# oharari/Convex-Combination-of-Gaussian-Processes

Measured on AMD Instinct MI355X. Metric: GP log-lik evals/sec (n x n fp64, batched over hyperpar grid), higher is better.
Workload: dtype f64; 1 GPU; cfg4: synthetic maximin-LHS 5-D design n=4096, K=3 anisotropic components, 512-point hyperparameter grid sharded over the GPUs; n=4096, d=5, K=3, evals_total=512, evals_per_gpu=512, parallelism=grid sharded over 1 GPU(s), one all-gather

## Files before the change

convex-combination-of-gaussian-processes_amd/csrc/blocked.hip:

```cpp
#include <cstdlib>
#include <vector>

#include "ccgp_internal.h"
#include "sched_logic.h"

namespace ccgp {

typedef double d4 __attribute__((ext_vector_type(4)));

namespace {

__device__ __forceinline__ int tid_now() {
  int t = threadIdx.x;
  asm volatile("" : "+v"(t));
  return t;
}

__device__ __forceinline__ constexpr int swz_src(int l, int parity) { return (((l >> 3) ^ parity) << 4) + ((l & 7) << 1); }

struct GemmArgs {
  double* A;
  size_t a_stride;
  int npad;
  double* invd;
  size_t invd_stride;
  int j, nt, nb;
  int ld;
  int ne;
  int extra_lower;
  int mode;
  double* E;
  size_t e_stride;
  int lde;
  int rows_only;
  int fuse_diag;
  int tail_strips;
  int wide;
  int n_s1;
  int tail_s;
  double* logdet_part;
  int* status;
  int n;
  double ptol;
};

template <int S, bool THIN>
struct TileGeom {
  static constexpr int CW = kTile / S;
  static constexpr int NX = THIN ? (S == 1 ? 2 : 1) : (S == 1 ? 4 : 2);
  static constexpr int NY = THIN ? 1 : (S == 4 ? 2 : 4);
  static constexpr int BK = 16;
  __device__ static int row0(int wave) { return THIN ? 0 : (S == 4 ? wave * 32 : (wave >> 1) * 64); }
  __device__ static int col0(int wave) {
    return THIN ? wave * NX * 16 : (S == 4 ? 0 : (wave & 1) * (S == 1 ? 64 : 32));
  }
};

template <int S, bool THIN, bool TRI>
__device__ __forceinline__ int col_block(int wave, int x) {
  if constexpr (TRI && !THIN) return (wave & 1) + 2 * x;
  else return (TileGeom<S, THIN>::col0(wave) >> 4) + x;
}

template <bool IL>
struct AccMap {
  int row0, col0, l15, l4;
  __device__ __forceinline__ AccMap() {
    const int lane = tid_now() & 63, wave = tid_now() >> 6;
    row0 = TileGeom<1, false>::row0(wave); col0 = TileGeom<1, false>::col0(wave); l15 = lane & 15; l4 = lane >> 4;
  }
  __device__ __forceinline__ int row(int y) const { return IL ? row0 + 4 * l15 + y : row0 + 16 * y + l15; }
  __device__ __forceinline__ int col(int x, int r) const { return IL ? col0 + 16 * r + 4 * l4 + x : col0 + 16 * x + l4 + 4 * r; }
  static constexpr __device__ __forceinline__ int dcol(int x, int r) { return IL ? 16 * r + x : 16 * x + 4 * r; }
  __device__ __forceinline__ double* lane_base(double* C, int ld) const {
    return IL ? C + row0 + 4 * l15 + (size_t)(col0 + 4 * l4) * ld : C + row0 + l15 + (size_t)(col0 + l4) * ld;
  }
};

template <int S, bool THIN, bool TRI = false>
__device__ __forceinline__ void gemm_accumulate(double* smem, const double* P, int ldP, const double* Q,
                                                int ldQ, int Kdim,
                                                d4 (&acc)[TileGeom<S, THIN>::NX][TileGeom<S, THIN>::NY]) {
  static_assert(!TRI || S == 1, "the triangular skip is only wired for full-width tiles");
  constexpr int CW = TileGeom<S, THIN>::CW;
  constexpr int NX = TileGeom<S, THIN>::NX;
  constexpr int NY = TileGeom<S, THIN>::NY;
  constexpr int BKs = TileGeom<S, THIN>::BK;
  constexpr int STAGE = BKs * kTile + BKs * CW;
  constexpr int CPI = kTile / CW;
  constexpr int QI = BKs / CPI / 4;
  const int tid = tid_now(), lane = tid & 63, wave = tid >> 6;
  const int row0 = TileGeom<S, THIN>::row0(wave);
  const int col0 = TileGeom<S, THIN>::col0(wave);
  const bool active = !THIN || col0 < CW;
  const int l15 = lane & 15, l4 = lane >> 4;

#pragma unroll
  for (int x = 0; x < NX; ++x)
#pragma unroll
    for (int y = 0; y < NY; ++y) acc[x][y] = d4{0.0, 0.0, 0.0, 0.0};

  const double* pP = P + swz_src(lane, wave & 1) + (size_t)wave * ldP;
  const size_t stepP = (size_t)4 * ldP;
  constexpr int LPC = 64 / CPI;
  const int qcol_in = lane / LPC, ql = lane % LPC;
  const int qpar = CPI == 1 ? (wave & 1) : (qcol_in & 1);
  const double* pQ = Q + swz_src(ql, qpar) + (size_t)(CPI * wave + qcol_in) * ldQ;
  const size_t stepQ = (size_t)(4 * CPI) * ldQ;

  auto issue = [&](int stage) {
    double* Ps_ = smem + stage * STAGE + wave * kTile;
    double* Qs_ = smem + stage * STAGE + BKs * kTile + wave * kTile;
#pragma unroll
    for (int q = 0; q < BKs / 4; ++q)
      __builtin_amdgcn_global_load_lds((const __attribute__((address_space(1))) void*)(pP + q * stepP),
                                       (__attribute__((address_space(3))) void*)(Ps_ + 4 * q * kTile), 16, 0, 0);
#pragma unroll
    for (int q = 0; q < QI; ++q)
      __builtin_amdgcn_global_load_lds((const __attribute__((address_space(1))) void*)(pQ + q * stepQ),
                                       (__attribute__((address_space(3))) void*)(Qs_ + 4 * q * kTile), 16, 0, 0);
    pP += (BKs / 4) * stepP;
    pQ += QI * stepQ;
  };

  static_assert(BKs == 16, "the pipeline below is written for four k-steps per stage");
  double pfA[NY], qfA[NX], pfB[NY], qfB[NX];
  const int sw = l4 & 1;
#define CCGP_LOADF(PF, QF, STG, KK)                                                              \
  do {                                                                                          \
    const double* Ps_ = smem + (STG) * STAGE;                                                   \
    const double* Qs_ = Ps_ + BKs * kTile;                                                      \
    _Pragma("unroll") for (int y = 0; y < NY; ++y)                                              \
        PF[y] = Ps_[((KK) * 4 + l4) * kTile + ((((row0 >> 4) + y) ^ sw) << 4) + l15];           \
    _Pragma("unroll") for (int x = 0; x < NX; ++x)                                              \
        QF[x] = Qs_[((KK) * 4 + l4) * CW + ((col_block<S, THIN, TRI>(wave, x) ^ sw) << 4) + l15]; \
    __builtin_amdgcn_sched_barrier(0);                                                          \
  } while (0)
#define CCGP_MFMAS(PF, QF, KT, X0, X1)                                                           \
  do {                                                                                          \
    if (active) {                                                                               \
      _Pragma("unroll") for (int x = (X0); x < (X1); ++x) {                                     \
        if (TRI && col_block<S, THIN, TRI>(wave, x) * 16 + 15 < (KT) * BKs) continue;           \
        _Pragma("unroll") for (int y = 0; y < NY; ++y)                                          \
            acc[x][y] = __builtin_amdgcn_mfma_f64_16x16x4f64(QF[x], PF[y], acc[x][y], 0, 0, 0); \
      }                                                                                         \
    }                                                                                           \
    __builtin_amdgcn_sched_barrier(0);                                                          \
  } while (0)
  constexpr int XH = NX > 1 ? 1 : NX;

  const int nk = Kdim / BKs;
  issue(0);
  __syncthreads();
  if (nk > 1) issue(1);
  CCGP_LOADF(pfA, qfA, 0, 0);
  for (int kt = 0; kt < nk; ++kt) {
    const int stg = kt & 1;
    CCGP_MFMAS(pfA, qfA, kt, 0, XH);
    CCGP_LOADF(pfB, qfB, stg, 1);
    CCGP_MFMAS(pfA, qfA, kt, XH, NX);
    CCGP_MFMAS(pfB, qfB, kt, 0, XH);
    CCGP_LOADF(pfA, qfA, stg, 2);
    CCGP_MFMAS(pfB, qfB, kt, XH, NX);
    CCGP_MFMAS(pfA, qfA, kt, 0, XH);
    CCGP_LOADF(pfB, qfB, stg, 3);
    CCGP_MFMAS(pfA, qfA, kt, XH, NX);
    if (kt + 1 < nk) {
      __syncthreads();
      if (kt + 2 < nk) issue(stg);
    }
    CCGP_MFMAS(pfB, qfB, kt, 0, XH);
// ... 201 lines not shown
#pragma unroll
        for (int t = 0; t < 2; ++t)
#pragma unroll
          for (int r = 0; r < 4; ++r) Co[t * 16 + (size_t)(gr.cb * 16 + 4 * r) * ld] = o[gr.cb][t][r];
      }
      __builtin_amdgcn_sched_barrier(0);
    }
  };
  struct Half0 { SolveGroup v[26]; };
  struct Half1 { SolveGroup v[10]; };
  constexpr Half0 h0{{{0, 0}, {1, 0}, {1, 1}, {2, 0}, {2, 1}, {2, 2}, {3, 0}, {3, 1}, {3, 2}, {3, 3},
                      {4, 0}, {4, 1}, {4, 2}, {4, 3}, {5, 0}, {5, 1}, {5, 2}, {5, 3},
                      {6, 0}, {6, 1}, {6, 2}, {6, 3}, {7, 0}, {7, 1}, {7, 2}, {7, 3}}};
  constexpr Half1 h1{{{4, 4}, {5, 4}, {5, 5}, {6, 4}, {6, 5}, {6, 6}, {7, 4}, {7, 5}, {7, 6}, {7, 7}}};

  __syncthreads();
  if ((wave & 1) == 0) dump();
  __syncthreads();
  run(h0, 0);
  __syncthreads();
  if ((wave & 1) == 1) dump();
  __syncthreads();
  run(h1, 1);
}

template <int S>
__device__ __forceinline__ void strip_accumulate_ring(double* smem, const double* P, int ldP, const double* Q, int ldQ,
                                                      int Kdim,
                                                      d4 (&acc)[TileGeom<S, false>::NX][TileGeom<S, false>::NY]) {
  static_assert(S == 2 || S == 4, "the ring exists for half- and quarter-width strips");
  constexpr int BKd = 8, NST = 4;
  constexpr int CW = TileGeom<S, false>::CW, NX = TileGeom<S, false>::NX, NY = TileGeom<S, false>::NY;
  static_assert(NX == 2, "the stage loop below splits a k-step's MFMAs at x = 1");
  constexpr int STAGE = BKd * kTile + BKd * CW;
  const int tid = tid_now(), lane = tid & 63, wave = tid >> 6;
  const int row0 = TileGeom<S, false>::row0(wave), col0 = TileGeom<S, false>::col0(wave);
  const int l15 = lane & 15, l4 = lane >> 4;
#pragma unroll
  for (int x = 0; x < NX; ++x)
#pragma unroll
    for (int y = 0; y < NY; ++y) acc[x][y] = d4{0.0, 0.0, 0.0, 0.0};

  const double* pP = P + swz_src(lane, wave & 1) + (size_t)wave * ldP;
  constexpr int LPR = CW / 2;
  const int ql = lane & (LPR - 1), qrow = lane / LPR;
  const int qw = S == 2 ? wave : (wave & 1);
  const double* pQ = Q + swz_src(ql, qrow & 1) + (size_t)(S * qw + qrow) * ldQ;
  auto issue = [&](int slot) {
    double* Ps_ = smem + slot * STAGE + wave * kTile;
    double* Qs_ = smem + slot * STAGE + BKd * kTile + qw * S * CW;
    __builtin_amdgcn_global_load_lds((const __attribute__((address_space(1))) void*)pP,
                                     (__attribute__((address_space(3))) void*)Ps_, 16, 0, 0);
    __builtin_amdgcn_global_load_lds((const __attribute__((address_space(1))) void*)(pP + (size_t)4 * ldP),
                                     (__attribute__((address_space(3))) void*)(Ps_ + 4 * kTile), 16, 0, 0);
    __builtin_amdgcn_global_load_lds((const __attribute__((address_space(1))) void*)pQ,
                                     (__attribute__((address_space(3))) void*)Qs_, 16, 0, 0);
    pP += (size_t)BKd * ldP;
    pQ += (size_t)BKd * ldQ;
  };
  auto wait_and_meet = [&](int later_stages) {
    if (later_stages >= 3) __builtin_amdgcn_s_waitcnt(0x0079);
    else if (later_stages == 2) __builtin_amdgcn_s_waitcnt(0x0076);
    else if (later_stages == 1) __builtin_amdgcn_s_waitcnt(0x0073);
    else __builtin_amdgcn_s_waitcnt(0x0070);
    __builtin_amdgcn_s_barrier();
  };

  const int sw = l4 & 1;
  const int offP = l4 * kTile + l15, offQ = BKd * kTile + l4 * CW + l15;
  int rbo[NY], cbo[NX];
#pragma unroll
  for (int t = 0; t < NY; ++t) rbo[t] = (((row0 >> 4) + t) ^ sw) << 4;
#pragma unroll
  for (int t = 0; t < NX; ++t) cbo[t] = (((col0 >> 4) + t) ^ sw) << 4;
  double pfA[NY], qfA[NX], pfB[NY], qfB[NX];
#define CCGP_RLOADF(PF, QF, SLOT, KK)                                                            \
  do {                                                                                          \
    const double* St_ = smem + (SLOT) * STAGE;                                                  \
    _Pragma("unroll") for (int y = 0; y < NY; ++y) PF[y] = St_[(KK) * 4 * kTile + offP + rbo[y]]; \
    _Pragma("unroll") for (int x = 0; x < NX; ++x) QF[x] = St_[(KK) * 4 * CW + offQ + cbo[x]];  \
    __builtin_amdgcn_sched_barrier(0);                                                          \
  } while (0)
#define CCGP_RMFMAS(PF, QF, X0, X1)                                                              \
  do {                                                                                          \
    _Pragma("unroll") for (int x = (X0); x < (X1); ++x)                                         \
      _Pragma("unroll") for (int y = 0; y < NY; ++y)                                            \
          acc[x][y] = __builtin_amdgcn_mfma_f64_16x16x4f64(QF[x], PF[y], acc[x][y], 0, 0, 0);   \
    __builtin_amdgcn_sched_barrier(0);                                                          \
  } while (0)

  const int nk = Kdim / BKd;
  const int pre = nk < NST ? nk : NST;
  for (int t = 0; t < pre; ++t) issue(t);
  __builtin_amdgcn_sched_barrier(0);
  wait_and_meet(pre - 1);
  CCGP_RLOADF(pfA, qfA, 0, 0);
  for (int kt = 0; kt < nk; ++kt) {
    const int slot = kt & (NST - 1);
    CCGP_RLOADF(pfB, qfB, slot, 1);
    CCGP_RMFMAS(pfA, qfA, 0, 2);
    if (kt + 1 < nk) {
      const int last_issued = kt + NST - 1 < nk - 1 ? kt + NST - 1 : nk - 1;
      wait_and_meet(last_issued - (kt + 1));
      if (kt + NST < nk) issue(slot);
      __builtin_amdgcn_sched_barrier(0);
    }
    CCGP_RMFMAS(pfB, qfB, 0, 1);
    if (kt + 1 < nk) CCGP_RLOADF(pfA, qfA, (kt + 1) & (NST - 1), 0);
    CCGP_RMFMAS(pfB, qfB, 1, 2);
  }
#undef CCGP_RLOADF
#undef CCGP_RMFMAS
}

template <int S, bool THIN, bool TRI = false, bool RING = false>
__device__ __forceinline__ void gemm_tile(double* smem, const double* P, int ldP, const double* Q,
                                          int ldQ, int Kdim, double* C, int ld, int mode) {
  constexpr int NX = TileGeom<S, THIN>::NX;
  constexpr int NY = TileGeom<S, THIN>::NY;
  d4 acc[NX][NY];
  if constexpr (RING) {
    static_assert((S == 2 || S == 4) && !THIN && !TRI, "the four-stage ring exists for half- and quarter-width update strips");
    strip_accumulate_ring<S>(smem, P, ldP, Q, ldQ, Kdim, acc);
  } else {
    gemm_accumulate<S, THIN, TRI>(smem, P, ldP, Q, ldQ, Kdim, acc);
  }
  const int lane = tid_now() & 63, wave = tid_now() >> 6;
  const int row0 = TileGeom<S, THIN>::row0(wave), col0 = TileGeom<S, THIN>::col0(wave);
  const int l15 = lane & 15, l4 = lane >> 4;
  if (THIN && col0 >= TileGeom<S, THIN>::CW) return;
#pragma unroll
  for (int x = 0; x < NX; ++x) {
    double cv[NY][4];
    if (mode == 0) {
#pragma unroll
      for (int y = 0; y < NY; ++y)
#pragma unroll
        for (int r = 0; r < 4; ++r)
          cv[y][r] = C[row0 + y * 16 + l15 + (size_t)(col_block<S, THIN, TRI>(wave, x) * 16 + l4 + 4 * r) * ld];
    }
#pragma unroll
    for (int y = 0; y < NY; ++y)
#pragma unroll
      for (int r = 0; r < 4; ++r) {
        double* p = C + row0 + y * 16 + l15 + (size_t)(col_block<S, THIN, TRI>(wave, x) * 16 + l4 + 4 * r) * ld;
        *p = mode == 0 ? cv[y][r] - acc[x][y][r] : acc[x][y][r];
      }
  }
}


template <int W>
__device__ __forceinline__ void diag_rhs_accumulate(double* smem, const double* Qp, const double* Tp, int ld,
                                                    int Kdim, d4 (&acc)[11]) {
  constexpr int BKs = 16, TR = 16, STAGE = BKs * kTile + BKs * TR;
  constexpr int RA = W, RB = 7 - W;
  constexpr int CBMAX = RA > RB ? RA : RB;
  constexpr bool XTRA = 2 * W + 1 > CBMAX;
  constexpr int NQ = CBMAX + 1 + (XTRA ? 2 : 0);
  constexpr int NR = W < 2 ? 5 : 4;
  auto frag_of = [](int cb) constexpr { return cb <= CBMAX ? cb : CBMAX + 1 + (cb - 2 * W); };
  auto cb_of_frag = [](int f) constexpr { return f <= CBMAX ? f : 2 * W + (f - CBMAX - 1); };
  const int lane = tid_now() & 63, l15 = lane & 15, l4 = lane >> 4, sw = l4 & 1;

  const __amdgpu_buffer_rsrc_t rQ = __builtin_amdgcn_make_buffer_rsrc((void*)Qp, 0, -1, 0x00020000);
  const __amdgpu_buffer_rsrc_t rT = __builtin_amdgcn_make_buffer_rsrc((void*)Tp, 0, -1, 0x00020000);
  const unsigned lane_q = (unsigned)(swz_src(lane, W & 1) * 8);
  const unsigned lane_t = (unsigned)((((lane & 7) << 1) + (size_t)(lane >> 3) * ld) * 8);
  const unsigned stepQ = (unsigned)ld * 32;
  unsigned oQ = (unsigned)W * (unsigned)ld * 8, oT = (unsigned)(8 * W) * (unsigned)ld * 8;
  auto request = [&](int stage, int r) {
    double* St_ = smem + stage * STAGE;
    if (r < 4)
      __builtin_amdgcn_raw_ptr_buffer_load_lds(rQ, (__attribute__((address_space(3))) void*)(St_ + (W + 4 * r) * kTile),
                                               16, lane_q, oQ + (unsigned)r * stepQ, 0, 0);
    else
      __builtin_amdgcn_raw_ptr_buffer_load_lds(rT, (__attribute__((address_space(3))) void*)(St_ + BKs * kTile + W * 8 * TR),
                                               16, lane_t, oT, 0, 0);
  };
  auto advance = [&]() { oQ += 4 * stepQ; oT += (unsigned)BKs * (unsigned)ld * 8; };

  int off[NQ];
#pragma unroll
  for (int f = 0; f < NQ; ++f) off[f] = l4 * kTile + ((cb_of_frag(f) ^ sw) << 4) + l15;
  const int offT = BKs * kTile + l4 * TR + l15;
  double fA[NQ + 1], fB[NQ + 1];
#define CCGP_SB __builtin_amdgcn_sched_barrier(0)
#define CCGP_DLOAD1(F, STG, KK, I)                                                                \
  do {                                                                                           \
    const double* St_ = smem + (STG) * STAGE;                                                    \
    if ((I) < NQ) F[I] = St_[(KK) * 4 * kTile + off[(I) < NQ ? (I) : 0]];                        \
    else F[NQ] = St_[(KK) * 4 * TR + offT];                                                      \
  } while (0)
#define CCGP_DSTEP(Fc, Fn, STGn, KKn, LD, RQ, STGr)                                               \
  do {                                                                                           \
    _Pragma("unroll") for (int s_ = 0; s_ < 11; ++s_) {                                          \
      const int cb_ = s_ >= 9 ? 2 * W + (s_ - 9) : (s_ <= W ? s_ : s_ - W - 1);                  \
      const double pf_ = s_ >= 9 ? Fc[NQ] : (s_ <= W ? Fc[frag_of(RA)] : Fc[frag_of(RB)]);       \
      acc[s_] = __builtin_amdgcn_mfma_f64_16x16x4f64(Fc[frag_of(cb_)], pf_, acc[s_], 0, 0, 0);   \
      if ((LD) && s_ <= NQ) CCGP_DLOAD1(Fn, STGn, KKn, s_);                                      \
      if ((RQ) && s_ < NR) request(STGr, s_);                                                    \
      CCGP_SB;                                                                                   \
    }                                                                                            \
  } while (0)
#define CCGP_DSTAGE(MORE, REFILL)                                                                 \
  do {                                                                                           \
    const int stg = kt & 1;                                                                      \
    CCGP_DSTEP(fA, fB, stg, 1, true, false, 0);                                                  \
    CCGP_DSTEP(fB, fA, stg, 2, true, false, 0);                                                  \
    CCGP_DSTEP(fA, fB, stg, 3, true, false, 0);                                                  \
    if (MORE) {                                                                                  \
      __syncthreads();                                                                           \
      CCGP_SB;                                                                                   \
    }                                                                                            \
    CCGP_DSTEP(fB, fA, stg ^ 1, 0, MORE, REFILL, stg);                                           \
    if (REFILL) advance();                                                                       \
  } while (0)

  const int nk = Kdim / BKs;
#pragma unroll
  for (int r = 0; r < NR; ++r) request(0, r);
  advance();
  __syncthreads();
  if (nk > 1) {
#pragma unroll
    for (int r = 0; r < NR; ++r) request(1, r);
    advance();
  }
#pragma unroll
  for (int i = 0; i <= NQ; ++i) CCGP_DLOAD1(fA, 0, 0, i);
  CCGP_SB;
  int kt = 0;
  for (; kt < nk - 2; ++kt) CCGP_DSTAGE(true, true);
  if (nk >= 2) { CCGP_DSTAGE(true, false); ++kt; }
  CCGP_DSTAGE(false, false);
#undef CCGP_DSTAGE
#undef CCGP_DSTEP
#undef CCGP_DLOAD1
#undef CCGP_SB
}

__device__ __forceinline__ void diag_rhs_accumulate_wide(double* smem, const double* Qp, const double* Tp, int ld,
                                                         int Kdim, int lane, int wave, const int (&cbs)[11],
                                                         d4 (&acc)[11]) {
  constexpr int BKs = 16, TR = 16, STAGE = BKs * kTile + BKs * TR, NS = 11;
  const int l15 = lane & 15, l4 = lane >> 4;
  const int rA = wave, rB = 7 - wave;
  const double* pQ = Qp + swz_src(lane, wave & 1) + (size_t)wave * ld;
  const double* pT = Tp + ((lane & 7) << 1) + (size_t)(8 * wave + (lane >> 3)) * ld;
  const size_t stepQ = (size_t)4 * ld;

  auto issue = [&](int stage) {
    double* Qs_ = smem + stage * STAGE + wave * kTile;
#pragma unroll
    for (int q = 0; q < BKs / 4; ++q)
      __builtin_amdgcn_global_load_lds((const __attribute__((address_space(1))) void*)(pQ + q * stepQ),
                                       (__attribute__((address_space(3))) void*)(Qs_ + 4 * q * kTile), 16, 0, 0);
    if (wave < 2)
      __builtin_amdgcn_global_load_lds((const __attribute__((address_space(1))) void*)pT,
                                       (__attribute__((address_space(3))) void*)(smem + stage * STAGE + BKs * kTile +
                                                                                 wave * 8 * TR),
                                       16, 0, 0);
    pQ += (BKs / 4) * stepQ;
    pT += (size_t)BKs * ld;
  };

  const int sw = l4 & 1;
  const int offA = l4 * kTile + ((rA ^ sw) << 4) + l15;
  const int offB = l4 * kTile + ((rB ^ sw) << 4) + l15;
  const int offT = BKs * kTile + l4 * TR + l15;
  int offQ[NS];
#pragma unroll
  for (int s = 0; s < NS; ++s) offQ[s] = l4 * kTile + ((cbs[s] ^ sw) << 4) + l15;

  double pfA[3], qfA[NS], pfB[3], qfB[NS];
#define CCGP_DLOADF(PF, QF, STG, KK)                                                             \
  do {                                                                                          \
    const double* St_ = smem + (STG) * STAGE;                                                   \
    PF[0] = St_[(KK) * 4 * kTile + offA];                                                       \
    PF[1] = St_[(KK) * 4 * kTile + offB];                                                       \
    PF[2] = St_[(KK) * 4 * TR + offT];                                                          \
    _Pragma("unroll") for (int s = 0; s < NS; ++s) QF[s] = St_[(KK) * 4 * kTile + offQ[s]];     \
    __builtin_amdgcn_sched_barrier(0);                                                          \
  } while (0)
#define CCGP_DMFMAS(PF, QF, S0, S1)                                                              \
  do {                                                                                          \
    _Pragma("unroll") for (int s = (S0); s < (S1); ++s) {                                       \
      const double pf = s >= 9 ? PF[2] : (s <= wave ? PF[0] : PF[1]);                           \
      acc[s] = __builtin_amdgcn_mfma_f64_16x16x4f64(QF[s], pf, acc[s], 0, 0, 0);                \
    }                                                                                           \
    __builtin_amdgcn_sched_barrier(0);                                                          \
  } while (0)
  constexpr int SH = 3;

  const int nk = Kdim / BKs;
  issue(0);
  __syncthreads();
  if (nk > 1) issue(1);
  CCGP_DLOADF(pfA, qfA, 0, 0);
  for (int kt = 0; kt < nk; ++kt) {
    const int stg = kt & 1;
    CCGP_DMFMAS(pfA, qfA, 0, SH);
    CCGP_DLOADF(pfB, qfB, stg, 1);
    CCGP_DMFMAS(pfA, qfA, SH, NS);
    CCGP_DMFMAS(pfB, qfB, 0, SH);
    CCGP_DLOADF(pfA, qfA, stg, 2);
    CCGP_DMFMAS(pfB, qfB, SH, NS);
    CCGP_DMFMAS(pfA, qfA, 0, SH);
    CCGP_DLOADF(pfB, qfB, stg, 3);
    CCGP_DMFMAS(pfA, qfA, SH, NS);
    if (kt + 1 < nk) {
      __syncthreads();
      if (kt + 2 < nk) issue(stg);
    }
    CCGP_DMFMAS(pfB, qfB, 0, SH);
    if (kt + 1 < nk) CCGP_DLOADF(pfA, qfA, stg ^ 1, 0);
    CCGP_DMFMAS(pfB, qfB, SH, NS);
  }
#undef CCGP_DLOADF
#undef CCGP_DMFMAS
}

__device__ __forceinline__ void diag_rhs_tile(double* smem, const double* Qp, const double* Tp, int ld,
                                              int Kdim, double* C, double* Ct, int wide) {
  constexpr int NS = 11;
  const int tid = tid_now(), lane = tid & 63;
  const int wave = __builtin_amdgcn_readfirstlane(tid >> 6);
  const int l15 = lane & 15, l4 = lane >> 4;
  const int rA = wave, rB = 7 - wave;

  d4 acc[NS];
#pragma unroll
  for (int s = 0; s < NS; ++s) acc[s] = d4{0.0, 0.0, 0.0, 0.0};

  int cbs[NS];
#pragma unroll
  for (int s = 0; s < 9; ++s) cbs[s] = s <= wave ? s : s - wave - 1;
  cbs[9] = 2 * wave;
  cbs[10] = 2 * wave + 1;

  if (!wide && fits_buffer_offsets(Kdim, ld)) {
    switch (wave) {
      case 0: diag_rhs_accumulate<0>(smem, Qp, Tp, ld, Kdim, acc); break;
      case 1: diag_rhs_accumulate<1>(smem, Qp, Tp, ld, Kdim, acc); break;
      case 2: diag_rhs_accumulate<2>(smem, Qp, Tp, ld, Kdim, acc); break;
      default: diag_rhs_accumulate<3>(smem, Qp, Tp, ld, Kdim, acc); break;
    }
  } else {
    diag_rhs_accumulate_wide(smem, Qp, Tp, ld, Kdim, lane, wave, cbs, acc);
  }

#pragma unroll
  for (int g0 = 0; g0 < NS; g0 += 4) {
    double cv[4][4];
#pragma unroll
    for (int u = 0; u < 4; ++u) {
      const int s = g0 + u;
      if (s >= NS) break;
      const int rb = s >= 9 ? 0 : (s <= wave ? rA : rB);
      double* base = s >= 9 ? Ct : C;
#pragma unroll
      for (int r = 0; r < 4; ++r) cv[u][r] = base[rb * 16 + l15 + (size_t)(cbs[s] * 16 + l4 + 4 * r) * ld];
    }
#pragma unroll
    for (int u = 0; u < 4; ++u) {
      const int s = g0 + u;
      if (s >= NS) break;
      const int rb = s >= 9 ? 0 : (s <= wave ? rA : rB);
      double* base = s >= 9 ? Ct : C;
#pragma unroll
      for (int r = 0; r < 4; ++r)
        base[rb * 16 + l15 + (size_t)(cbs[s] * 16 + l4 + 4 * r) * ld] = cv[u][r] - acc[s][r];
    }
  }
}

template <int S>
constexpr size_t gemm_lds_bytes() {
  return sizeof(double) * 2 * TileGeom<S, false>::BK * (kTile + kTile / S);
}

struct DiagArgs {
  double* A;
  size_t a_stride;
  int npad;
  double* invd;
  size_t invd_stride;
  double* logdet_part;
  int* status;
  int j, nt, nb, n;
  int ld;
  double ptol;
};

__host__ __device__ inline DiagArgs diag_args(const GemmArgs& g, int j) {
  return DiagArgs{g.A, g.a_stride, g.npad, g.invd, g.invd_stride, g.logdet_part, g.status, j, g.nt, g.nb, g.n, g.ld, g.ptol};
}

constexpr int kDiagLdsDoubles = 2 * 256 + kTile + 4;
__device__ __forceinline__ void diag_factor(const DiagArgs& g, int b, double* lds) {
  double (*colbuf)[256] = reinterpret_cast<double (*)[256]>(lds);
  double* dvec = lds + 2 * 256;
  double* red = dvec + kTile;
  const int tid = tid_now(), ty = tid & 15, tx = tid >> 4;
  const int ld = g.ld;
  double* C = g.A + (size_t)b * g.a_stride + (size_t)g.j * kTile + (size_t)g.j * kTile * ld;
  const double kNaN = __longlong_as_double(0x7ff8000000000000LL);

  double M[8][8];
  double I[8][8];
#pragma unroll
  for (int bb = 0; bb < 8; ++bb)
#pragma unroll
    for (int a = 0; a < 8; ++a) {
      const int r = ty + 16 * a, c = tx + 16 * bb;
      if (a >= bb) M[a][bb] = r >= c ? C[r + (size_t)c * ld] : 0.0;
      if (bb >= a) I[a][bb] = r == c ? 1.0 : 0.0;
    }

  int bad = 0, cur = 0;
#pragma unroll
  for (int kb = 0; kb < 8; ++kb) {
    for (int kk = 0; kk < 16; ++kk) {
      if (bad) break;
      const int k = 16 * kb + kk;
      if (tx == kk) {
#pragma unroll
        for (int a = kb; a < 8; ++a) colbuf[cur][ty + 16 * a] = M[a][kb];
#pragma unroll
        for (int a = 0; a <= kb; ++a) colbuf[cur][kTile + ty + 16 * a] = I[a][kb];
      }
      __syncthreads();
      const double piv = colbuf[cur][k];
      if (!(piv > g.ptol)) { bad = k + 1; break; }
      double rinv = __builtin_amdgcn_rcp(piv);
      rinv = fma(fma(-piv, rinv, 1.0), rinv, rinv);
      rinv = fma(fma(-piv, rinv, 1.0), rinv, rinv);
      if (tid == 0) dvec[k] = piv;
      double lc[8], lr[8], li[8];
#pragma unroll
      for (int bb = kb; bb < 8; ++bb) lc[bb] = colbuf[cur][tx + 16 * bb] * rinv;
      if (tx <= kk) lc[kb] = 0.0;
#pragma unroll
      for (int a = kb; a < 8; ++a) lr[a] = colbuf[cur][ty + 16 * a];
      if (ty <= kk) lr[kb] = 0.0;
#pragma unroll
      for (int a = 0; a <= kb; ++a) li[a] = colbuf[cur][kTile + ty + 16 * a];
#pragma unroll
      for (int bb = kb; bb < 8; ++bb) {
#pragma unroll
        for (int a = bb; a < 8; ++a) M[a][bb] = fma(-lr[a], lc[bb], M[a][bb]);
#pragma unroll
        for (int a = 0; a <= kb; ++a) I[a][bb] = fma(-li[a], lc[bb], I[a][bb]);
      }
      cur ^= 1;
    }
  }
  __syncthreads();

  double lsum = 0.0;
  if (!bad && tid < kTile) lsum = log(dvec[tid]);
  for (int off = 32; off > 0; off >>= 1) lsum += __shfl_down(lsum, off, 64);
  if ((tid & 63) == 0) red[tid >> 6] = lsum;
  __syncthreads();
  if (tid == 0) {
    g.logdet_part[(size_t)b * g.nt + g.j] = bad ? kNaN : (red[0] + red[1] + red[2] + red[3]);
    if (bad && g.status[b] == 0) g.status[b] = g.j * kTile + bad;
  }

  double* W = g.invd + (size_t)b * g.invd_stride + (size_t)g.j * kTile * kTile;
#pragma unroll
  for (int bb = 0; bb < 8; ++bb) {
    const int c = tx + 16 * bb;
    const double dc = bad ? 1.0 : dvec[c];
    const double sq = sqrt(dc), rs = 1.0 / sq;
#pragma unroll
    for (int a = 0; a < 8; ++a) {
      const int r = ty + 16 * a;
      if (a >= bb) {
        double v = r > c ? M[a][bb] * rs : (r == c ? sq : 0.0);
        C[r + (size_t)c * ld] = bad ? kNaN : v;
      }
      double w = 0.0;
      if (bb >= a) w = c >= r ? I[a][bb] * rs : 0.0;
      W[c + (size_t)r * kTile] = bad ? kNaN : w;
    }
  }
}

__global__ __launch_bounds__(256) void diag_kernel(DiagArgs g) {
  __shared__ double lds[kDiagLdsDoubles];
  diag_factor(g, blockIdx.x, lds);
}

__host__ __device__ inline int gemm_units_per_matrix(int mode, int nt, int j, int ne, int S, int rows_only = 0) {
  if (rows_only) return mode == 0 ? ne * S : ne;
  return mode == 0 ? 1 + ((nt - 1 - j) + ne) * S : (nt - j) + ne;
}

template <int MODE, int S>
__device__ __forceinline__ void gemm_unit(const GemmArgs& g, double* smem, int j, int b, int i, int strip, bool ring) {
  const int ld = g.ld;
  double* Ab = g.A + (size_t)b * g.a_stride;
  const bool thin = i == g.nt;
  const int c0 = strip * (ring ? kTile / g.tail_s : kTile / S);

  int k0 = 0;
  if (g.extra_lower && i > g.nt) {
    const int te = i - g.nt - 1;
    if (j < te || (MODE == 0 && j == te)) return;
    k0 = te * kTile;
  }
  double* rowbase = Ab + (size_t)i * kTile;
  int rld = ld;
  if (g.E && i > g.nt) {
    rowbase = g.E + (size_t)b * g.e_stride + (size_t)(i - g.nt - 1) * kTile;
    rld = g.lde;
  }
  const double* P;
  const double* Q;
  int ldP, ldQ, Kdim;
  if (MODE == 0) {
    P = rowbase + (size_t)k0 * rld;
    Q = Ab + (size_t)j * kTile + c0 + (size_t)k0 * ld;
    ldP = rld;
    ldQ = ld;
    Kdim = j * kTile - k0;
  } else {
    P = rowbase + (size_t)j * kTile * rld;
    Q = g.invd + (size_t)b * g.invd_stride + (size_t)j * kTile * kTile + c0;
    ldP = rld;
    ldQ = kTile;
    Kdim = kTile;
  }
  double* C = rowbase + ((size_t)j * kTile + c0) * rld;
  constexpr bool TRI = MODE == 1 && S == 1;
  if constexpr (MODE == 1) {
    if (thin) { gemm_tile<S, true, TRI>(smem, P, ldP, Q, ldQ, Kdim, C, rld, MODE); return; }
  }
  if constexpr (MODE == 0 && S == 1) {
    if (ring) {
      if (g.tail_s == 4) gemm_tile<4, false, false, true>(smem, P, ldP, Q, ldQ, Kdim, C, rld, MODE);
      else gemm_tile<2, false, false, true>(smem, P, ldP, Q, ldQ, Kdim, C, rld, MODE);
      return;
    }
    if (!g.wide && fits_buffer_offsets(Kdim, ldP > ldQ ? ldP : ldQ)) {
      update_tile_il(smem, P, ldP, Q, ldQ, Kdim, C, rld);
      return;
    }
  }
  gemm_tile<S, false, TRI>(smem, P, ldP, Q, ldQ, Kdim, C, rld, MODE);
}

__device__ __forceinline__ void diag_unit(const GemmArgs& g, double* smem, int j, int b) {
  const int ld = g.ld;
  double* Ab = g.A + (size_t)b * g.a_stride;
  diag_rhs_tile(smem, Ab + (size_t)j * kTile, Ab + g.npad, ld, j * kTile,
                Ab + (size_t)j * kTile + (size_t)j * kTile * ld, Ab + g.npad + (size_t)j * kTile * ld, g.wide);
  if (g.fuse_diag) {
    __syncthreads();
    diag_factor(diag_args(g, j), b, smem);
  }
}

template <int MODE, int S>
__device__ __forceinline__ void gemm_dispatch(const GemmArgs& g, double* smem) {
  const int L = blockIdx.x;
  int b, i, strip = 0;
  bool ring = false;
  if (MODE == 0 && !g.rows_only) {
    const int nb8 = (g.nb + 7) & ~7;
    if (L < nb8) {
      if (L < g.nb) diag_unit(g, smem, g.j, L);
      return;
    }
    const int nfull = (g.nt - 1 - g.j) + g.ne;
    const int Lt = L - nb8;
    int u1;
    if (S == 1) {
      if (Lt >= g.n_s1) {
        const int q = Lt - g.n_s1;
        u1 = g.n_s1 + ((q / (8 * g.tail_s)) << 3) + (q & 7);
        strip = (q >> 3) % g.tail_s;
        ring = true;
      } else {
        u1 = Lt;
      }
    } else {
      u1 = ((Lt / (8 * S)) << 3) + (Lt & 7);
      strip = (Lt >> 3) % S;
    }
    const int per_grp = 8 * nfull;
    const int grp = u1 / per_grp, r = u1 % per_grp;
    b = grp * 8 + (r & 7);
    if (b >= g.nb) return;
    i = g.j + 1 + (r >> 3);
    if (i >= g.nt) i += 1;
  } else {
    const int per_grp = 8 * gemm_units_per_matrix(MODE, g.nt, g.j, g.ne, S, g.rows_only);
    const int grp = L / per_grp, r = L % per_grp;
    b = grp * 8 + (r & 7);
    if (b >= g.nb) return;
    const int u = r >> 3;
    if (g.rows_only) {
      strip = MODE == 0 ? u % S : 0;
      i = g.nt + 1 + (MODE == 0 ? u / S : u);
    } else {
      i = g.j + 1 + u;
    }
  }
  gemm_unit<MODE, S>(g, smem, g.j, b, i, strip, ring);
}

#define CCGP_DEFINE_GEMM(NAME, MODE, S, WPS)                                            \
  __global__ __launch_bounds__(256, WPS) void NAME(GemmArgs g) {                        \
    extern __shared__ __attribute__((aligned(16))) double smem[];                       \
    gemm_dispatch<MODE, S>(g, smem);                                                     \
  }
CCGP_DEFINE_GEMM(chol_update_kernel, 0, 1, 2)
CCGP_DEFINE_GEMM(chol_update_s2_kernel, 0, 2, 2)
CCGP_DEFINE_GEMM(chol_trsm_kernel, 1, 1, 2)
#undef CCGP_DEFINE_GEMM

__global__ __launch_bounds__(256, 2) void chol_diag_solve_kernel(GemmArgs g) {
  extern __shared__ __attribute__((aligned(16))) double smem[];
  const int b = blockIdx.x;
  if (b >= g.nb) return;
  diag_unit(g, smem, g.j, b);
  __syncthreads();
  gemm_unit<1, 1>(g, smem, g.j, b, g.nt, 0, false);
}

__global__ __launch_bounds__(256, 2) void chol_update_solve_kernel(GemmArgs g) {
  extern __shared__ __attribute__((aligned(16))) double smem[];
  const int per_grp = 8 * (g.nt - 1 - g.j);
  const int grp = blockIdx.x / per_grp, r = blockIdx.x % per_grp;
  const int b = grp * 8 + (r & 7);
  if (b >= g.nb) return;
  const int i = g.j + 1 + (r >> 3), ld = g.ld;
  double* Ab = g.A + (size_t)b * g.a_stride;
  update_solve_tile_il(smem, Ab + (size_t)i * kTile, ld, Ab + (size_t)g.j * kTile, ld, g.j * kTile,
                       Ab + (size_t)i * kTile + (size_t)g.j * kTile * ld, ld,
                       g.invd + (size_t)b * g.invd_stride + (size_t)g.j * kTile * kTile);
}

#include "blocked_sched.inc"


static int update_tail(int nb8, int tiles, int quarters, int* ts) {
  const long w1 = (long)nb8 * (1 + tiles), all_tiles = (long)nb8 * tiles;
  const long rem = w1 % 256;
  *ts = 2;
  if (rem == 0 || all_tiles == 0) return 0;
  long tail = rem < all_tiles ? rem : all_tiles;
  if (tail != rem && w1 > 256) return 0;
  if (quarters && w1 > 256 && (rem - tail) + 4 * tail <= 512) { *ts = 4; return (int)tail; }
  if (rem + tail > 256) return 0;
  return (int)tail;
}

static void launch_gemm(hipStream_t s, GemmArgs g, int mode, int S) {
  const int nb8 = round_up(g.nb, 8);
  int units = nb8 * gemm_units_per_matrix(mode, g.nt, g.j, g.ne, S, g.rows_only);
  if (mode == 0 && !g.rows_only) {
    const int tiles = (g.nt - 1 - g.j) + g.ne;
    int ts = 2;
    const int tail = (S == 1 && g.tail_strips) ? update_tail(nb8, tiles, g.tail_strips == 1, &ts) : 0;
    g.n_s1 = nb8 * tiles - tail;
    g.tail_s = ts;
    units = nb8 + (S == 1 ? g.n_s1 + ts * tail : nb8 * tiles * S);
  }
  const dim3 grid(units), block(256);
  if (mode == 0) {
    if (S == 1) hipLaunchKernelGGL(chol_update_kernel, grid, block, gemm_lds_bytes<1>(), s, g);
    else hipLaunchKernelGGL(chol_update_s2_kernel, grid, block, gemm_lds_bytes<2>(), s, g);
  } else {
    hipLaunchKernelGGL(chol_trsm_kernel, grid, block, gemm_lds_bytes<1>(), s, g);
  }
}

struct RhsArgs {
  double* A;
  size_t a_stride;
  int npad, n;
  const double* y;
  int ld;
  int identity;
};

__global__ __launch_bounds__(256) void rhs_rows_kernel(RhsArgs g) {
  const int ld = g.ld;
  double* Ab = g.A + (size_t)blockIdx.y * g.a_stride;
  const int c = blockIdx.x * 16 + (threadIdx.x >> 4);
  const int r = threadIdx.x & 15;
  double v = 0.0;
  if (c < g.n) v = r == 0 ? g.y[c] : (r == 1 ? 1.0 : 0.0);
  Ab[g.npad + r + (size_t)c * ld] = v;
  const int e_end = g.identity ? min(ld, g.npad + kTile + (c / kTile + 1) * kTile) : ld;
  for (int e = g.npad + kTile + r; e < e_end; e += 16)
    Ab[e + (size_t)c * ld] = (g.identity && e - (g.npad + kTile) == c) ? 1.0 : 0.0;
}

struct FinishArgs {
  const double* A;
  size_t a_stride;
  int npad;
  const double* logdet_part;
  const double* params;
  int ldp, K;
  int b0, nt, n;
  double sigma2;
  int mode;
  double* loglik;
  double* beta;
  const int* status;
  int ld;
  double* s11_out;
  double* beta_out;
  double* logdet_out;
  double* s2hat;
  double* q_out;
};

__device__ inline double block_sum(double v, double* red, int tid) {
  for (int off = 32; off > 0; off >>= 1) v += __shfl_down(v, off, 64);
  __syncthreads();
  if ((tid & 63) == 0) red[tid >> 6] = v;
  __syncthreads();
  return red[0] + red[1] + red[2] + red[3];
}

template <bool PROF = false>
__global__ __launch_bounds__(256) void finish_kernel(FinishArgs g) {
  __shared__ double red[4];
  const int b = blockIdx.x, tid = threadIdx.x;
  const int ld = g.ld;
  const double* zrow = g.A + (size_t)b * g.a_stride + g.npad;
  double logdet = 0.0;
  for (int jb = tid; jb < g.nt; jb += 256) logdet += g.logdet_part[(size_t)b * g.nt + jb];
  logdet = block_sum(logdet, red, tid);
  double s11 = 0.0, s1y = 0.0, syy = 0.0;
  for (int c = tid; c < g.n; c += 256) {
    const double zy = zrow[(size_t)c * ld], z1 = zrow[1 + (size_t)c * ld];
    s11 = fma(z1, z1, s11);
    s1y = fma(z1, zy, s1y);
    syy = fma(zy, zy, syy);
  }
  s11 = block_sum(s11, red, tid);
  s1y = block_sum(s1y, red, tid);
  syy = block_sum(syy, red, tid);
  const double kLog2Pi = 1.8378770664093454835606594728112;
  const int gb = g.b0 + b;
  double sw = 0.0;
  for (int c = 0; c < g.K; ++c) { double w = g.params[gb + (size_t)c * g.ldp]; sw += w * w; }
  const double cs = g.sigma2 * sw;
  double beta = 0.0, ll;
  if (g.mode == 0) {
    beta = s1y / s11;
    double q = 0.0;
    for (int c = tid; c < g.n; c += 256) {
      const double v = zrow[(size_t)c * ld] - beta * zrow[1 + (size_t)c * ld];
      q = fma(v, v, q);
    }
    q = block_sum(q, red, tid);
    if (tid == 0 && g.q_out) g.q_out[gb] = (g.status && g.status[gb] != 0) ? __longlong_as_double(0x7ff8000000000000LL) : q;
    if constexpr (PROF) {
      const double csh = q / g.n;
      ll = -0.5 * (g.n * kLog2Pi + g.n * log(csh) + logdet + g.n);
      if (tid == 0) g.s2hat[gb] = (g.status && g.status[gb] != 0) ? __longlong_as_double(0x7ff8000000000000LL) : csh / sw;
    } else {
      ll = -0.5 * (g.n * kLog2Pi + g.n * log(cs) + logdet + q / cs);
    }
  } else {
    ll = -0.5 * (g.n * kLog2Pi + logdet + syy);
  }
  if (tid == 0) {
    const double kNaN = __longlong_as_double(0x7ff8000000000000LL);
    if (g.status && g.status[gb] != 0) { ll = kNaN; beta = kNaN; }
    if (g.loglik) g.loglik[gb] = ll;
    if (g.beta) g.beta[gb] = beta;
    if (g.s11_out) g.s11_out[b] = s11;
    if (g.logdet_out) g.logdet_out[gb] = (g.status && g.status[gb] != 0) ? kNaN : logdet;
    if (g.beta_out) g.beta_out[b] = beta;
// ... 684 lines not shown
```

Measured before the change: 2617 evals/s.

## Compute thin RHS block with per-lane FMAs and fuse thin triangular solve

New measurement: 2633 evals/s (median of 6 runs). About the same (+0.6%).

```diff
diff --git a/convex-combination-of-gaussian-processes_amd/csrc/blocked.hip b/convex-combination-of-gaussian-processes_amd/csrc/blocked.hip
--- a/convex-combination-of-gaussian-processes_amd/csrc/blocked.hip
+++ b/convex-combination-of-gaussian-processes_amd/csrc/blocked.hip
@@ -2,6 +2,7 @@
 #include <vector>
 
 #include "ccgp_internal.h"
+#include "rhs_lane_map.h"
 #include "sched_logic.h"
 
 namespace ccgp {
@@ -16,7 +17,7 @@
   return t;
 }
 
-__device__ __forceinline__ constexpr int swz_src(int l, int parity) { return (((l >> 3) ^ parity) << 4) + ((l & 7) << 1); }
+static_assert(kRhsPanelW == kTile, "rhs_lane_map.h describes the 128-wide panel image");
 
 struct GemmArgs {
   double* A;
@@ -524,15 +525,12 @@
 
 template <int W>
 __device__ __forceinline__ void diag_rhs_accumulate(double* smem, const double* Qp, const double* Tp, int ld,
-                                                    int Kdim, d4 (&acc)[11]) {
-  constexpr int BKs = 16, TR = 16, STAGE = BKs * kTile + BKs * TR;
+                                                    int Kdim, d4 (&acc)[9], double& z) {
+  constexpr int BKs = kRhsStageK, TR = kRhsRowsW, STAGE = BKs * kTile + BKs * TR;
   constexpr int RA = W, RB = 7 - W;
-  constexpr int CBMAX = RA > RB ? RA : RB;
-  constexpr bool XTRA = 2 * W + 1 > CBMAX;
-  constexpr int NQ = CBMAX + 1 + (XTRA ? 2 : 0);
+  constexpr int NQ = (RA > RB ? RA : RB) + 1;
   constexpr int NR = W < 2 ? 5 : 4;
-  auto frag_of = [](int cb) constexpr { return cb <= CBMAX ? cb : CBMAX + 1 + (cb - 2 * W); };
-  auto cb_of_frag = [](int f) constexpr { return f <= CBMAX ? f : 2 * W + (f - CBMAX - 1); };
+  constexpr int ZF = 8;
   const int lane = tid_now() & 63, l15 = lane & 15, l4 = lane >> 4, sw = l4 & 1;
 
   const __amdgpu_buffer_rsrc_t rQ = __builtin_amdgcn_make_buffer_rsrc((void*)Qp, 0, -1, 0x00020000);
@@ -554,23 +552,27 @@
 
   int off[NQ];
 #pragma unroll
-  for (int f = 0; f < NQ; ++f) off[f] = l4 * kTile + ((cb_of_frag(f) ^ sw) << 4) + l15;
-  const int offT = BKs * kTile + l4 * TR + l15;
-  double fA[NQ + 1], fB[NQ + 1];
+  for (int f = 0; f < NQ; ++f) off[f] = l4 * kTile + ((f ^ sw) << 4) + l15;
+  const int zq0 = rhs_q_offset(W, lane, 0), zq1 = rhs_q_offset(W, lane, 1) - kTile, zt0 = BKs * kTile + rhs_t_offset(lane, 0);
+  double fA[NQ], fB[NQ], zA[8], zB[8];
 #define CCGP_SB __builtin_amdgcn_sched_barrier(0)
-#define CCGP_DLOAD1(F, STG, KK, I)                                                                \
+#define CCGP_DLOAD1(F, STG, KK, I) F[I] = (smem + (STG) * STAGE)[(KK) * 4 * kTile + off[I]]
+#define CCGP_ZLOAD1(Z, STG, KK, U)                                                                \
   do {                                                                                           \
     const double* St_ = smem + (STG) * STAGE;                                                    \
-    if ((I) < NQ) F[I] = St_[(KK) * 4 * kTile + off[(I) < NQ ? (I) : 0]];                        \
-    else F[NQ] = St_[(KK) * 4 * TR + offT];                                                      \
+    if ((U) < 4) Z[U] = St_[((KK) * 4 + ((U) & 3)) * kTile + (((U) & 1) ? zq1 : zq0)];           \
+    else Z[U] = St_[((KK) * 4 + ((U) & 3)) * TR + zt0];                                          \
   } while (0)
-#define CCGP_DSTEP(Fc, Fn, STGn, KKn, LD, RQ, STGr)                                               \
+#define CCGP_DSTEP(Fc, Fn, Zc, Zn, STGn, KKn, LD, RQ, STGr)                                       \
   do {                                                                                           \
-    _Pragma("unroll") for (int s_ = 0; s_ < 11; ++s_) {                                          \
-      const int cb_ = s_ >= 9 ? 2 * W + (s_ - 9) : (s_ <= W ? s_ : s_ - W - 1);                  \
-      const double pf_ = s_ >= 9 ? Fc[NQ] : (s_ <= W ? Fc[frag_of(RA)] : Fc[frag_of(RB)]);       \
-      acc[s_] = __builtin_amdgcn_mfma_f64_16x16x4f64(Fc[frag_of(cb_)], pf_, acc[s_], 0, 0, 0);   \
-      if ((LD) && s_ <= NQ) CCGP_DLOAD1(Fn, STGn, KKn, s_);                                      \
+    _Pragma("unroll") for (int s_ = 0; s_ < 9; ++s_) {                                           \
+      const int cb_ = s_ <= W ? s_ : s_ - W - 1;                                                 \
+      acc[s_] = __builtin_amdgcn_mfma_f64_16x16x4f64(Fc[cb_], s_ <= W ? Fc[RA] : Fc[RB], acc[s_], 0, 0, 0); \
+      if ((LD) && s_ < NQ) CCGP_DLOAD1(Fn, STGn, KKn, s_);                                       \
+      if ((LD) && s_ < 8) CCGP_ZLOAD1(Zn, STGn, KKn, s_);                                        \
+      if (s_ == ZF) {                                                                            \
+        _Pragma("unroll") for (int i_ = 0; i_ < 4; ++i_) z = __builtin_fma(Zc[4 + i_], Zc[i_], z); \
+      }                                                                                          \
       if ((RQ) && s_ < NR) request(STGr, s_);                                                    \
       CCGP_SB;                                                                                   \
     }                                                                                            \
@@ -578,14 +580,14 @@
 #define CCGP_DSTAGE(MORE, REFILL)                                                                 \
   do {                                                                                           \
     const int stg = kt & 1;                                                                      \
-    CCGP_DSTEP(fA, fB, stg, 1, true, false, 0);                                                  \
-    CCGP_DSTEP(fB, fA, stg, 2, true, false, 0);                                                  \
-    CCGP_DSTEP(fA, fB, stg, 3, true, false, 0);                                                  \
+    CCGP_DSTEP(fA, fB, zA, zB, stg, 1, true, false, 0);                                          \
+    CCGP_DSTEP(fB, fA, zB, zA, stg, 2, true, false, 0);                                          \
+    CCGP_DSTEP(fA, fB, zA, zB, stg, 3, true, false, 0);                                          \
     if (MORE) {                                                                                  \
       __syncthreads();                                                                           \
       CCGP_SB;                                                                                   \
     }                                                                                            \
-    CCGP_DSTEP(fB, fA, stg ^ 1, 0, MORE, REFILL, stg);                                           \
+    CCGP_DSTEP(fB, fA, zB, zA, stg ^ 1, 0, MORE, REFILL, stg);                                   \
     if (REFILL) advance();                                                                       \
   } while (0)
 
@@ -600,7 +602,9 @@
     advance();
   }
 #pragma unroll
-  for (int i = 0; i <= NQ; ++i) CCGP_DLOAD1(fA, 0, 0, i);
+  for (int i = 0; i < NQ; ++i) CCGP_DLOAD1(fA, 0, 0, i);
+#pragma unroll
+  for (int u = 0; u < 8; ++u) CCGP_ZLOAD1(zA, 0, 0, u);
   CCGP_SB;
   int kt = 0;
   for (; kt < nk - 2; ++kt) CCGP_DSTAGE(true, true);
@@ -608,6 +612,7 @@
   CCGP_DSTAGE(false, false);
 #undef CCGP_DSTAGE
 #undef CCGP_DSTEP
+#undef CCGP_ZLOAD1
 #undef CCGP_DLOAD1
 #undef CCGP_SB
 }
@@ -693,58 +698,69 @@
 #undef CCGP_DMFMAS
 }
 
-__device__ __forceinline__ void diag_rhs_tile(double* smem, const double* Qp, const double* Tp, int ld,
-                                              int Kdim, double* C, double* Ct, int wide) {
-  constexpr int NS = 11;
+template <int NS>
+__device__ __forceinline__ void diag_rhs_store(const d4 (&acc)[NS], int wave, int lane, double* C, double* Ct, int ld) {
+  const int l15 = lane & 15, l4 = lane >> 4;
+  auto elem = [&](int s, int r) -> double* {
+    const int cb = s >= 9 ? 2 * wave + (s - 9) : (s <= wave ? s : s - wave - 1);
+    const int rb = s >= 9 ? 0 : (s <= wave ? wave : 7 - wave);
+    return (s >= 9 ? Ct : C) + rb * 16 + l15 + (size_t)(cb * 16 + l4 + 4 * r) * ld;
+  };
+#pragma unroll
+  for (int g0 = 0; g0 < NS; g0 += 4) {
+    double cv[4][4];
+#pragma unroll
+    for (int u = 0; u < 4; ++u) {
+      if (g0 + u >= NS) break;
+#pragma unroll
+      for (int r = 0; r < 4; ++r) cv[u][r] = *elem(g0 + u, r);
+    }
+#pragma unroll
+    for (int u = 0; u < 4; ++u) {
+      if (g0 + u >= NS) break;
+#pragma unroll
+      for (int r = 0; r < 4; ++r) *elem(g0 + u, r) = cv[u][r] - acc[g0 + u][r];
+    }
+  }
+}
+
+__device__ __forceinline__ bool diag_rhs_tile(double* smem, const double* Qp, const double* Tp, int ld,
+                                              int Kdim, double* C, double* Ct, int wide, double* t_keep) {
   const int tid = tid_now(), lane = tid & 63;
   const int wave = __builtin_amdgcn_readfirstlane(tid >> 6);
-  const int l15 = lane & 15, l4 = lane >> 4;
-  const int rA = wave, rB = 7 - wave;
-
+
+  if (!wide && fits_buffer_offsets(Kdim, ld)) {
+    d4 acc[9];
+#pragma unroll
+    for (int s = 0; s < 9; ++s) acc[s] = d4{0.0, 0.0, 0.0, 0.0};
+    double z = 0.0;
+    switch (wave) {
+      case 0: diag_rhs_accumulate<0>(smem, Qp, Tp, ld, Kdim, acc, z); break;
+      case 1: diag_rhs_accumulate<1>(smem, Qp, Tp, ld, Kdim, acc, z); break;
+      case 2: diag_rhs_accumulate<2>(smem, Qp, Tp, ld, Kdim, acc, z); break;
+      default: diag_rhs_accumulate<3>(smem, Qp, Tp, ld, Kdim, acc, z); break;
+    }
+    double* pz = Ct + rhs_lane_row(lane) + (size_t)rhs_lane_col(wave, lane) * ld;
+    const double cz = *pz;
+    diag_rhs_store<9>(acc, wave, lane, C, Ct, ld);
+    const double tz = cz - z;
+    *pz = tz;
+    if (t_keep) t_keep[rhs_lane_row(lane) * kTile + rhs_lane_col(wave, lane)] = tz;
+    return t_keep != nullptr;
+  }
+
+  constexpr int NS = 11;
   d4 acc[NS];
+  int cbs[NS];
 #pragma unroll
   for (int s = 0; s < NS; ++s) acc[s] = d4{0.0, 0.0, 0.0, 0.0};
-
-  int cbs[NS];
 #pragma unroll
   for (int s = 0; s < 9; ++s) cbs[s] = s <= wave ? s : s - wave - 1;
   cbs[9] = 2 * wave;
   cbs[10] = 2 * wave + 1;
-
-  if (!wide && fits_buffer_offsets(Kdim, ld)) {
-    switch (wave) {
-      case 0: diag_rhs_accumulate<0>(smem, Qp, Tp, ld, Kdim, acc); break;
-      case 1: diag_rhs_accumulate<1>(smem, Qp, Tp, ld, Kdim, acc); break;
-      case 2: diag_rhs_accumulate<2>(smem, Qp, Tp, ld, Kdim, acc); break;
-      default: diag_rhs_accumulate<3>(smem, Qp, Tp, ld, Kdim, acc); break;
-    }
-  } else {
-    diag_rhs_accumulate_wide(smem, Qp, Tp, ld, Kdim, lane, wave, cbs, acc);
-  }
-
-#pragma unroll
-  for (int g0 = 0; g0 < NS; g0 += 4) {
-    double cv[4][4];
-#pragma unroll
-    for (int u = 0; u < 4; ++u) {
-      const int s = g0 + u;
-      if (s >= NS) break;
-      const int rb = s >= 9 ? 0 : (s <= wave ? rA : rB);
-      double* base = s >= 9 ? Ct : C;
-#pragma unroll
-      for (int r = 0; r < 4; ++r) cv[u][r] = base[rb * 16 + l15 + (size_t)(cbs[s] * 16 + l4 + 4 * r) * ld];
-    }
-#pragma unroll
-    for (int u = 0; u < 4; ++u) {
-      const int s = g0 + u;
-      if (s >= NS) break;
-      const int rb = s >= 9 ? 0 : (s <= wave ? rA : rB);
-      double* base = s >= 9 ? Ct : C;
-#pragma unroll
-      for (int r = 0; r < 4; ++r)
-        base[rb * 16 + l15 + (size_t)(cbs[s] * 16 + l4 + 4 * r) * ld] = cv[u][r] - acc[s][r];
-    }
-  }
+  diag_rhs_accumulate_wide(smem, Qp, Tp, ld, Kdim, lane, wave, cbs, acc);
+  diag_rhs_store<NS>(acc, wave, lane, C, Ct, ld);
+  return false;
 }
 
 template <int S>
@@ -924,15 +940,16 @@
   gemm_tile<S, false, TRI>(smem, P, ldP, Q, ldQ, Kdim, C, rld, MODE);
 }
 
-__device__ __forceinline__ void diag_unit(const GemmArgs& g, double* smem, int j, int b) {
+__device__ __forceinline__ bool diag_unit(const GemmArgs& g, double* smem, int j, int b, double* t_keep = nullptr) {
   const int ld = g.ld;
   double* Ab = g.A + (size_t)b * g.a_stride;
-  diag_rhs_tile(smem, Ab + (size_t)j * kTile, Ab + g.npad, ld, j * kTile,
-                Ab + (size_t)j * kTile + (size_t)j * kTile * ld, Ab + g.npad + (size_t)j * kTile * ld, g.wide);
+  const bool kept = diag_rhs_tile(smem, Ab + (size_t)j * kTile, Ab + g.npad, ld, j * kTile, Ab + (size_t)j * kTile + (size_t)j * kTile * ld,
+                                  Ab + g.npad + (size_t)j * kTile * ld, g.wide, t_keep);
   if (g.fuse_diag) {
     __syncthreads();
     diag_factor(diag_args(g, j), b, smem);
   }
+  return kept;
 }
 
 template <int MODE, int S>
@@ -994,13 +1011,49 @@
 CCGP_DEFINE_GEMM(chol_trsm_kernel, 1, 1, 2)
 #undef CCGP_DEFINE_GEMM
 
+constexpr int kThinKeepOffset = 2 * (kRhsStageK * kTile + kRhsStageK * kRhsRowsW);
+static_assert(kThinKeepOffset >= kDiagLdsDoubles && (kThinKeepOffset + 2 * kTile) * sizeof(double) <= gemm_lds_bytes<1>(),
+              "the kept right-hand-side rows lie inside the launch's LDS and outside what diag_factor uses");
+__device__ __forceinline__ void thin_solve_lanes(const double* Tl, const double* Wj, double* Cz, int ld) {
+  const int tid = tid_now(), lane = tid & 63;
+  const int wave = __builtin_amdgcn_readfirstlane(tid >> 6);
+  const int r = rhs_lane_row(lane), c = rhs_lane_col(wave, lane), cb = c >> 4;
+  const double* w = Wj + c;
+  const double* t = Tl + r * kTile;
+  const int nkb = 2 * wave + 2;
+  double z = 0.0, wn[16];
+#pragma unroll
+  for (int i = 0; i < 16; ++i) wn[i] = w[(size_t)i * kTile];
+  for (int kb = 0; kb < nkb; ++kb) {
+    double wc[16];
+#pragma unroll
+    for (int i = 0; i < 16; ++i) wc[i] = wn[i];
+    if (kb + 1 < nkb) {
+#pragma unroll
+      for (int i = 0; i < 16; ++i) wn[i] = w[(size_t)((kb + 1) * 16 + i) * kTile];
+    }
+    if (kb <= cb) {
+#pragma unroll
+      for (int i = 0; i < 16; ++i) z = __builtin_fma(wc[i], t[kb * 16 + i], z);
+    }
+  }
+  Cz[r + (size_t)c * ld] = z;
+}
+
 __global__ __launch_bounds__(256, 2) void chol_diag_solve_kernel(GemmArgs g) {
   extern __shared__ __attribute__((aligned(16))) double smem[];
   const int b = blockIdx.x;
   if (b >= g.nb) return;
-  diag_unit(g, smem, g.j, b);
+  double* t_keep = smem + kThinKeepOffset;
+  const bool kept = diag_unit(g, smem, g.j, b, t_keep);
   __syncthreads();
-  gemm_unit<1, 1>(g, smem, g.j, b, g.nt, 0, false);
+  if (kept) {
+    double* Ab = g.A + (size_t)b * g.a_stride;
+    thin_solve_lanes(t_keep, g.invd + (size_t)b * g.invd_stride + (size_t)g.j * kTile * kTile,
+                     Ab + g.npad + (size_t)g.j * kTile * g.ld, g.ld);
+  } else {
+    gemm_unit<1, 1>(g, smem, g.j, b, g.nt, 0, false);
+  }
 }
 
 __global__ __launch_bounds__(256, 2) void chol_update_solve_kernel(GemmArgs g) {
diff --git a/convex-combination-of-gaussian-processes_amd/csrc/rhs_lane_map.h b/convex-combination-of-gaussian-processes_amd/csrc/rhs_lane_map.h
--- /dev/null
+++ b/convex-combination-of-gaussian-processes_amd/csrc/rhs_lane_map.h
@@ -0,0 +1,19 @@
+#pragma once
+
+namespace ccgp {
+
+constexpr int kRhsPanelW = 128;
+constexpr int kRhsRowsW = 16;
+constexpr int kRhsStageK = 16;
+
+constexpr int swz_src(int l, int parity) { return (((l >> 3) ^ parity) << 4) + ((l & 7) << 1); }
+
+constexpr int rhs_lane_row(int lane) { return lane >> 5; }
+constexpr int rhs_lane_col(int W, int lane) { return 32 * W + (lane & 31); }
+
+constexpr int rhs_q_offset(int W, int lane, int k) {
+  return k * kRhsPanelW + ((((rhs_lane_col(W, lane) >> 4) ^ (k & 1))) << 4) + (rhs_lane_col(W, lane) & 15);
+}
+constexpr int rhs_t_offset(int lane, int k) { return k * kRhsRowsW + rhs_lane_row(lane); }
+
+}
```
